# ttanida/rgrg

Hardware: AMD Instinct MI355X
Metric: images/sec full 29-region report gen, 512x512 CXR, greedy max_len=128 (higher is better)
Workload: dtype bf16; 1 GPU; full_model.generate() batch=32/GPU, 29 regions, greedy max_len=128, bf16 autocast: 16-bit detector, 16-bit decode GEMMs + K/V cache, hipGraph-captured decode step (BASELINE configs[2]); global_batch=32, parallelism=single GPU, weights=seeded random init (rgrg_amd.synth, profile bench), hipGraph_decode=True

## Files before the change

include/rgrg_hip.h:

```cpp
#ifndef RGRG_HIP_H_
#define RGRG_HIP_H_

#include <stdint.h>

#ifdef __cplusplus
extern "C" {
#endif

#define RGRG_OK 0
#define RGRG_EINVAL (-1)
#define RGRG_EHIP (-2)
#define RGRG_ESTATE (-3)

#define RGRG_ACT_NONE 0
#define RGRG_ACT_RELU 1
#define RGRG_ACT_GELU_NEW 2

const char* rgrg_last_error(void);
int rgrg_abi_version(void);
int rgrg_device_arch(int dev, char* buf, int buflen);

int rgrg_linear_f32(const float* A, const float* W, const float* scale, const float* shift, const float* R,
                    float* Y, int M, int N, int K, int ldy, int act, int splitk, float* ws, void* stream);
int rgrg_conv2d_nhwc_f32(const float* X, const float* W, const float* scale, const float* shift, const float* R,
// ... 68 lines not shown
                                  int* launches_per_step);
int rgrg_dropout_mask_f32(uint64_t seed, uint32_t stream_id, float p, int64_t n, int row_len, float* out, void* stream);
int rgrg_decoder_forward_cached(rgrg_decoder* d, const float* feats, const int64_t* input_ids, const int64_t* position_ids,
                                const float* attention_mask,
                                int S, int T, int past_len, float* logits_out, void* stream);
int rgrg_decoder_cache_plane(rgrg_decoder* d, int layer, int kv, void** ptr, int* max_seqs, int* slots, int* is_bf16);
int rgrg_decoder_take_id_error(rgrg_decoder* d, int* pending);
int rgrg_decoder_refresh_trainable(rgrg_decoder* d, void* stream);
int rgrg_transpose_pad_f32(const float* src, float* dst, int rows, int cols, int rows_padded, void* stream);
int rgrg_colsum_f32(const float* src, float* out, int rows, int cols, void* stream);
int rgrg_relu_backward_f32(float* d, const float* h, int64_t n, void* stream);
int rgrg_bce_with_logits_masked_backward_f32(const float* logits, const uint8_t* mask, const uint8_t* target, float pos_weight,
                                             int n, float scale, float* dlogits, int ld, void* stream);
int rgrg_adamw_step_f32(float* param, const float* grad, float* exp_avg, float* exp_avg_sq, int64_t n, float lr, float beta1,
                        float beta2, float eps, float weight_decay, int step, float grad_scale, void* stream);
int rgrg_adamw_multi_step_f32(const void* items, int n_items, float lr, float beta1, float beta2, float eps,
                              float weight_decay, int step, float grad_scale, void* stream);
int rgrg_f32_to_bf16(const float* src, uint16_t* dst, int64_t n, int fp16, void* stream);
int rgrg_bf16_to_f32(const uint16_t* src, float* dst, int64_t n, int fp16, void* stream);
int rgrg_conv2d_nhwc_bf16(const uint16_t* X16, const uint16_t* Wb, const float* shift, const uint16_t* R16, float* Y,
                          uint16_t* Y16, int B, int H, int Wd, int Cin, int Cout, int KH, int KW, int stride, int pad,
                          int act, int fp16, void* stream);
int rgrg_linear_bf16w_f32(const float* A, const uint16_t* Wb, const float* shift, const float* R, float* Y, int M,
                          int N, int K, int ldy, int act, int fp16, void* stream);
int rgrg_linear_bf16_f32(const uint16_t* A16, const uint16_t* Wb, const float* shift, const float* R, float* Y,
                         uint16_t* Y16, int M, int N, int K, int ldy, int act, int fp16, void* stream);
int rgrg_debug_linear_bf16_tile(const uint16_t* A16, const uint16_t* Wb, const float* shift, const float* R, float* Y,
                                int M, int N, int K, int ldy, int act, int tile, int lda, int ldw, int fp16, void* stream);
int rgrg_debug_linear_bf16_train(const uint16_t* A16, const uint16_t* Wb, const float* shift, const float* R, float* Y,
                                 uint16_t* Y16, uint16_t* Ypre16, const uint16_t* G16, int M, int N, int K, int ldy, int act,
                                 int tile, int fp16, void* stream);
int rgrg_debug_linear_bf16_argmax(const uint16_t* A16, const uint16_t* Wb, const float* shift, int M, int N, int K,
                                  float* cand_val, int* cand_idx, int fp16, void* stream);
int rgrg_debug_ln_fold16(const float* w, const float* gain, const float* beta, const float* bias, uint16_t* wb, float* colsum,
                         float* shift, int N, int K, int fp16, void* stream);
int rgrg_debug_linear_bf16_ln(const uint16_t* A16, const uint16_t* Wb, const float* shift, const float* R, float* Y,
                              uint16_t* Yb16, float* stats_out, const float* ln_stats, const float* ln_colsum, int M, int N,
                              int K, int ldy, int act, int fp16, void* stream);
int rgrg_debug_linear_bf16_ln_kp(const uint16_t* A16, const uint16_t* Wb, const float* shift, const float* R, float* Y,
                                 uint16_t* Y16, uint16_t* Yb16, float* stats_out, const float* ln_stats, const float* ln_colsum,
                                 int M, int N, int K, int ldy, int act, int fp16, int kp, void* stream);
int rgrg_box_match_f32(const float* gt, const int* gt_count, int G, const float* boxes, int64_t box_image_stride,
                       const int* box_count, int B, int N, float high, float low, int allow_low_quality, int* matched,
                       int* ws_best_per_gt, void* stream);
int rgrg_balanced_sample(const int* matched, const int64_t* gt_labels, int G, const int* box_count, const float* keys,
                         uint64_t seed, int stage, int B, int n, int batch, int max_pos, uint32_t* ws_keys, uint8_t* mask,
                         int* list, int* count, void* stream);
int rgrg_rpn_loss_sampled_f32(const float* rpn_out, int ld, int anchors_per_cell, const int* matched, const float* gt, int G,
                              const float* anchors, const uint8_t* mask, const int* list, const int* count, int B, int A,
                              int batch, float* out2, void* stream);
int rgrg_roi_add_gt_f32(const float* props, const int* counts, int P, const float* gt, const int* gt_count, int G, int B,
                        float* boxes, int* box_count, void* stream);
int rgrg_roi_gather_samples_f32(const float* boxes, const int* matched, const float* gt, const int64_t* gt_labels,
                                const int* gt_count, int G, const int* list, const int* count, int B, int N, int K, float wx,
                                float wy, float ww, float wh, float* props_s, int* offsets, int64_t* labels_flat,
                                float* reg_targets, void* stream);
int rgrg_fastrcnn_loss_f32(const float* pred, int ld, int num_classes, const int64_t* labels, const float* reg_targets, int N,
                           float* out2, void* stream);

int rgrg_decoder_copy_last_logits(rgrg_decoder* d, float* dst, int S, void* stream);
int rgrg_decoder_time_step_parts(rgrg_decoder* d, int S, int nkeys, int iters, int one_range, float* ms_gemm, float* ms_attn,
                                 double* gemm_flops, double* gemm_weight_bytes, double* kv_bytes, int* gemm_launches);
int rgrg_decoder_trace_step(rgrg_decoder* d, int S, int nkeys, int iters, float* recs, int max_recs, int* n_out);
int rgrg_decoder_attention_only(rgrg_decoder* d, int S, int nkeys, int iters, void* stream);
int rgrg_decoder_row_limit(rgrg_decoder* d);
int rgrg_debug_chain(int n, int mode, int blocks, float* us_per_kernel);
// ... 6 lines not shown
```

rgrg_amd/_hip.py:

```python
from __future__ import annotations

import ctypes as C
import os
from typing import Optional

from . import build as _build

c_float_p = C.c_void_p
_i, _f, _p = C.c_int, C.c_float, C.c_void_p

ACT_NONE, ACT_RELU, ACT_GELU_NEW = 0, 1, 2
ABI_VERSION = 21


class RgrgHipError(RuntimeError):
    pass


class DecoderLayerWeights(C.Structure):
    _fields_ = [(n, _p) for n in ("ln1_g", "ln1_b", "ln2_g", "ln2_b", "c_attn_w", "c_attn_b", "attn_proj_w",
                                  "attn_proj_b", "c_fc_w", "c_fc_b", "mlp_proj_w", "mlp_proj_b")]


class DecoderWeights(C.Structure):
# ... 16 lines not shown
    "rgrg_top1_per_class_f32": (_i, [_p, _i, _p, _p, _p, _p, _p, _p, _p, _i, _i, _i, _f, _f, _p]),
    "rgrg_select_regions_f32": (_i, [_p, _p, _f, _p, _p, _p, _i, _p]),
    "rgrg_bce_with_logits_masked_f32": (_i, [_p, _p, _p, C.c_float, _i, _p, _p]),
    "rgrg_preprocess_u8_f32": (_i, [_p, _i, _i, _i, _i, _i, C.c_float, C.c_float, _p, _p]),
    "rgrg_gather_rows_f32": (_i, [_p, _p, _p, _i, _i, _p]),
    "rgrg_decoder_create": (_i, [C.POINTER(DecoderWeights), _i, _i, C.POINTER(_p)]),
    "rgrg_decoder_create_with_cache": (_i, [C.POINTER(DecoderWeights), _i, _i, _p, C.c_size_t, C.POINTER(_p)]),
    "rgrg_decoder_kv_cache_bytes": (C.c_size_t, [_i, _i, _i]),
    "rgrg_decoder_destroy": (None, [_p]),
    "rgrg_decoder_generate": (_i, [_p, _p, _i, _i, _p, _i, C.POINTER(_i), _i, _p]),
    "rgrg_decoder_beam_search": (_i, [_p, _p, _i, _i, _i, _i, _f, _i, _p, _i, C.POINTER(_i), _p]),
    "rgrg_decoder_set_precision": (_i, [_p, _i]),
    "rgrg_decoder_lm_forward": (_i, [_p, _p, _p, _p, _i, _i, _p, _p, _p]),
    "rgrg_decoder_lm_loss_grad": (_i, [_p, _p, _p, _p, _i, _i, C.c_float, C.c_float, C.c_uint64, _p, _p, _p, _p, _p, _p, _p, _p]),
    "rgrg_dropout_mask_f32": (_i, [C.c_uint64, C.c_uint32, C.c_float, C.c_int64, _i, _p, _p]),
    "rgrg_decoder_refresh_trainable": (_i, [_p, _p]),
    "rgrg_decoder_take_id_error": (_i, [_p, C.POINTER(_i)]),
    "rgrg_decoder_forward_cached": (_i, [_p, _p, _p, _p, _p, _i, _i, _i, _p, _p]),
    "rgrg_decoder_cache_plane": (_i, [_p, _i, _i, C.POINTER(C.c_void_p), C.POINTER(_i), C.POINTER(_i), C.POINTER(_i)]),
    "rgrg_transpose_pad_f32": (_i, [_p, _p, _i, _i, _i, _p]),
    "rgrg_colsum_f32": (_i, [_p, _p, _i, _i, _p]),
    "rgrg_relu_backward_f32": (_i, [_p, _p, C.c_int64, _p]),
    "rgrg_bce_with_logits_masked_backward_f32": (_i, [_p, _p, _p, C.c_float, _i, C.c_float, _p, _i, _p]),
    "rgrg_adamw_step_f32": (_i, [_p, _p, _p, _p, C.c_int64, C.c_float, C.c_float, C.c_float, C.c_float, C.c_float, _i, C.c_float, _p]),
    "rgrg_adamw_multi_step_f32": (_i, [_p, _i, C.c_float, C.c_float, C.c_float, C.c_float, C.c_float, _i, C.c_float, _p]),
    "rgrg_f32_to_bf16": (_i, [_p, _p, C.c_int64, _i, _p]),
    "rgrg_bf16_to_f32": (_i, [_p, _p, C.c_int64, _i, _p]),
    "rgrg_conv2d_nhwc_bf16": (_i, [_p, _p, _p, _p, _p, _p, _i, _i, _i, _i, _i, _i, _i, _i, _i, _i, _i, _p]),
    "rgrg_linear_bf16w_f32": (_i, [_p, _p, _p, _p, _p, _i, _i, _i, _i, _i, _i, _p]),
    "rgrg_linear_bf16_f32": (_i, [_p, _p, _p, _p, _p, _p, _i, _i, _i, _i, _i, _i, _p]),
    "rgrg_debug_linear_bf16_tile": (_i, [_p, _p, _p, _p, _p, _i, _i, _i, _i, _i, _i, _i, _i, _i, _p]),
    "rgrg_debug_linear_bf16_train": (_i, [_p, _p, _p, _p, _p, _p, _p, _p, _i, _i, _i, _i, _i, _i, _i, _p]),
    "rgrg_debug_linear_bf16_argmax": (_i, [_p, _p, _p, _i, _i, _i, _p, _p, _i, _p]),
    "rgrg_debug_ln_fold16": (_i, [_p, _p, _p, _p, _p, _p, _p, _i, _i, _i, _p]),
    "rgrg_debug_linear_bf16_ln": (_i, [_p, _p, _p, _p, _p, _p, _p, _p, _p, _i, _i, _i, _i, _i, _i, _p]),
    "rgrg_debug_linear_bf16_ln_kp": (_i, [_p, _p, _p, _p, _p, _p, _p, _p, _p, _p, _i, _i, _i, _i, _i, _i, _i, _p]),
    "rgrg_decoder_copy_last_logits": (_i, [_p, _p, _i, _p]),
    "rgrg_box_match_f32": (_i, [_p, _p, _i, _p, C.c_int64, _p, _i, _i, _f, _f, _i, _p, _p, _p]),
    "rgrg_balanced_sample": (_i, [_p, _p, _i, _p, _p, C.c_uint64, _i, _i, _i, _i, _i, _p, _p, _p, _p, _p]),
    "rgrg_rpn_loss_sampled_f32": (_i, [_p, _i, _i, _p, _p, _i, _p, _p, _p, _p, _i, _i, _i, _p, _p]),
    "rgrg_roi_add_gt_f32": (_i, [_p, _p, _i, _p, _p, _i, _i, _p, _p, _p]),
    "rgrg_roi_gather_samples_f32": (_i, [_p, _p, _p, _p, _p, _i, _p, _p, _i, _i, _i, _f, _f, _f, _f, _p, _p, _p, _p, _p]),
    "rgrg_fastrcnn_loss_f32": (_i, [_p, _i, _i, _p, _p, _i, _p, _p]),
    "rgrg_decoder_trace_step": (_i, [_p, _i, _i, _i, _p, _i, C.POINTER(_i)]),
    "rgrg_decoder_attention_only": (_i, [_p, _i, _i, _i, _p]),
    "rgrg_decoder_row_limit": (_i, [_p]),
    "rgrg_decoder_set_lm_positions": (_i, [_p, _p, C.c_int64]),
    "rgrg_decoder_time_step_parts": (_i, [_p, _i, _i, _i, _i, C.POINTER(_f), C.POINTER(_f), C.POINTER(C.c_double),
                                          C.POINTER(C.c_double), C.POINTER(C.c_double), C.POINTER(_i)]),
    "rgrg_decoder_time_train_gemms": (_i, [_p, _i, _i, _i, C.POINTER(_f), C.POINTER(C.c_double), C.POINTER(_i)]),
    "rgrg_debug_chain": (_i, [_i, _i, _i, C.POINTER(_f)]),
}

_lib: Optional[C.CDLL] = None


def library_path() -> str:
    return _build.LIB_PATH


def load() -> C.CDLL:
    global _lib
    if _lib is not None:
        return _lib
    path = library_path()
    if _build.is_stale():
# ... 41 lines not shown
```

rgrg_amd/csrc/decoder.hip:

```cpp
#include <math.h>
#include <stdlib.h>

#include <algorithm>
#include <type_traits>
#include <cmath>
#include <vector>

#include "common.h"

namespace rgrg {

struct GemmParams;
int launch_gemm_dense(const float* A, const float* W, const float* shift, const float* R, float* Y, int M, int N, int K,
                      int ldy, int act, float* ws, size_t ws_floats, hipStream_t st);
int init_gemm_attrs();
int init_gemm_bf16_attrs();
struct GemmLnFold {
    void* Yb16 = nullptr;
    float* stats_out = nullptr;
    const float* ln_stats = nullptr;
    const float* ln_colsum = nullptr;
    void* Ypre16 = nullptr;
    const void* G16 = nullptr;
    int ksplit = 0;
    float* sk_ws = nullptr;
    unsigned* sk_cnt = nullptr;
    float* cand_val = nullptr;
    int* cand_idx = nullptr;
    int kp = 0;
};
bool gemm_bf16_cand_epilogue_ok(int M, int N, int K);
int launch_gemm_bf16w_ex(const float* A, const void* A16, const void* Wb, const float* shift, const float* R, float* Y, void* Y16,
                         int M, int N, int K, int ldy, int act, hipStream_t st, int f16, const GemmLnFold* ln = nullptr);
int launch_gemm_bf16w(const float* A, const void* Wb, const float* shift, const float* R, float* Y, int M, int N, int K,
                      int ldy, int act, hipStream_t st, int f16);
int convert_f32_to_bf16(const float* src, void* dst, size_t n, hipStream_t st, int f16);

constexpr int MAX_CHAINS = 4;
constexpr int PAD_ROWS = 32;
constexpr int SKINNY_MAX_ROWS = 128;
static int skinny_max_rows() {
    static int v = -1;
    if (v < 0) { const char* e = getenv("RGRG_SKINNY_MAX_ROWS"); v = e ? atoi(e) : SKINNY_MAX_ROWS;
        if (v > SKINNY_MAX_ROWS) v = SKINNY_MAX_ROWS; if (v < 32) v = 32; }
    return v;
}
constexpr int BOS_ID = 50256, EOS_ID = 50256, PAD_ID = 50256;
constexpr float LN_EPS = 1e-5f;

__global__ __launch_bounds__(256) void pack_weights_kernel(const float* __restrict__ W, float* __restrict__ P, int N,
                                                           int K, int NT) {
    const size_t total = (size_t)NT * (K / 8) * 64;
    for (size_t o = (size_t)blockIdx.x * blockDim.x + threadIdx.x; o < total; o += (size_t)gridDim.x * blockDim.x) {
        const int l = (int)(o & 63);
        const size_t t = o >> 6;
        const int kc = (int)(t % (K / 8));
        const int nt = (int)(t / (K / 8));
        const int n = nt * 32 + (l & 31);
        f32x4 v = {0.f, 0.f, 0.f, 0.f};
        if (n < N) v = *reinterpret_cast<const f32x4*>(W + (size_t)n * K + kc * 8 + (l >> 5) * 4);
        reinterpret_cast<f32x4*>(P)[o] = v;
    }
}

struct SkinnyArgs {
    const float* X;
    const float* P;
    const float* bias;
    const float* R;
    float* Y;
    float* part;
// ... 415 lines not shown
            L += pl[k] * wgt;
            o += pacc[k][threadIdx.x] * wgt;
        }
        out[frag_out ? frag_off(s, hd * 64 + threadIdx.x, D) : (size_t)s * D + hd * 64 + threadIdx.x] = o / L;
    }
}

typedef unsigned short u16;
typedef unsigned int u32x4 __attribute__((ext_vector_type(4)));
template <bool F16>
__device__ __forceinline__ float pair_lo(unsigned u) {
    if constexpr (F16) return f16_bits_to_f32(u & 0xffffu);
    else return __uint_as_float(u << 16);
}
template <bool F16>
__device__ __forceinline__ float pair_hi(unsigned u) {
    if constexpr (F16) return f16_bits_to_f32(u >> 16);
    else return __uint_as_float(u & 0xffff0000u);
}

struct Kv16Row {
    f32x4 q0, q1, k0, k1, v0, v1;
};
template <bool F16>
__device__ __forceinline__ u32x4 kv16_pack_round(const f32x4& lo, const f32x4& hi) {
    u32x4 o;
    o[0] = to16<F16>(lo[0]) | (to16<F16>(lo[1]) << 16);
    o[1] = to16<F16>(lo[2]) | (to16<F16>(lo[3]) << 16);
    o[2] = to16<F16>(hi[0]) | (to16<F16>(hi[1]) << 16);
    o[3] = to16<F16>(hi[2]) | (to16<F16>(hi[3]) << 16);
    return o;
}

template <int NI, bool HAS_SRC, bool FIRST, bool F16>
__device__ __forceinline__ void kv16_wave_chunk(const __amdgpu_buffer_rsrc_t kc, const __amdgpu_buffer_rsrc_t vc, const int* __restrict__ srow,
                                                int s, int hd, int H, int T, int base, int nkeys, int slot, int g, int d8,
                                                Kv16Row& r, float (&q)[8], u32x4& kn16, u32x4& vn16, float& m, float& l, float (&acc)[8]) {
    int rowi[NI];
#pragma unroll
    for (int i = 0; i < NI; ++i) rowi[i] = HAS_SRC ? srow[min(base + i * 8 + g, nkeys - 1)] : s;
    u32x4 kk[NI], vv[NI];
#pragma unroll
    for (int i = 0; i < NI; ++i) {
        const int jc = min(base + i * 8 + g, nkeys - 1);
        const unsigned off = ((unsigned)((rowi[i] * H + hd) * T + jc) * 64u + (unsigned)d8 * 8u) * 2u;
        kk[i] = __builtin_bit_cast(u32x4, __builtin_amdgcn_raw_buffer_load_b128(kc, (int)off, 0, 2));
        vv[i] = __builtin_bit_cast(u32x4, __builtin_amdgcn_raw_buffer_load_b128(vc, (int)off, 0, 2));
    }
    __builtin_amdgcn_sched_barrier(0);
    if constexpr (FIRST) {
#pragma unroll
        for (int e = 0; e < 4; ++e)
            asm volatile("" : "+v"(r.q0[e]), "+v"(r.q1[e]), "+v"(r.k0[e]), "+v"(r.k1[e]), "+v"(r.v0[e]), "+v"(r.v1[e]));
#pragma unroll
        for (int e = 0; e < 4; ++e) { q[e] = r.q0[e]; q[4 + e] = r.q1[e]; }
        kn16 = kv16_pack_round<F16>(r.k0, r.k1);
        vn16 = kv16_pack_round<F16>(r.v0, r.v1);
    }
    float sc[NI];
    float cmax = -INFINITY;
#pragma unroll
    for (int i = 0; i < NI; ++i) {
        const int j = base + i * 8 + g;
        if (j == slot) { kk[i] = kn16; vv[i] = vn16; }
        float dot = 0.f;
#pragma unroll
        for (int e = 0; e < 4; ++e)
            dot += q[2 * e] * pair_lo<F16>(kk[i][e]) + q[2 * e + 1] * pair_hi<F16>(kk[i][e]);
        dot += dpp_get<0xB1, 0xf>(dot);
        dot += dpp_get<0x4E, 0xf>(dot);
        dot += dpp_get<0x141, 0xf>(dot);
        sc[i] = j < nkeys ? dot / 8.0f : -INFINITY;
        cmax = fmaxf(cmax, sc[i]);
    }
    const float m_new = fmaxf(m, cmax);
    const float scale = (m == -INFINITY) ? 0.f : expf(m - m_new);
    const bool any = m_new != -INFINITY;
    l *= scale;
#pragma unroll
    for (int e = 0; e < 8; ++e) acc[e] *= scale;
#pragma unroll
    for (int i = 0; i < NI; ++i) {
        const int j = base + i * 8 + g;
        const float pj = (j < nkeys && any) ? expf(sc[i] - m_new) : 0.f;
        l += pj;
#pragma unroll
        for (int e = 0; e < 4; ++e) {
            const unsigned u = j < nkeys ? vv[i][e] : 0u;
            acc[2 * e] += pj * pair_lo<F16>(u);
            acc[2 * e + 1] += pj * pair_hi<F16>(u);
        }
    }
    m = m_new;
}

template <bool HAS_SRC, bool F16>
__global__ __launch_bounds__(256) void attn_decode_kv16_wave_kernel(const float* __restrict__ qkv, int ld_qkv,
                                                                    u16* __restrict__ kc, u16* __restrict__ vc,
                                                                    const int* __restrict__ step, float* __restrict__ out,
                                                                    int S, int H, int T, const int* __restrict__ src,
                                                                    u16* __restrict__ out16) {
    const int lane = threadIdx.x & 63;
    const int t = *step, nkeys = t + 2, slot = t + 1;
    const int g = lane >> 3, d8 = lane & 7;
    const int D = H * 64;
    const __amdgpu_buffer_rsrc_t rk = dx_rsrc(kc), rv = dx_rsrc(vc);
    for (int item = blockIdx.x * 4 + (threadIdx.x >> 6); item < S * H; item += gridDim.x * 4) {
    const int s = item / H, hd = item - s * H;
    const float* row = qkv + (size_t)s * ld_qkv;
    const int* srow = HAS_SRC ? src + (size_t)s * T : nullptr;
    Kv16Row r;
    r.q0 = *reinterpret_cast<const f32x4*>(row + hd * 64 + d8 * 8);
    r.q1 = *reinterpret_cast<const f32x4*>(row + hd * 64 + d8 * 8 + 4);
    r.k0 = *reinterpret_cast<const f32x4*>(row + D + hd * 64 + d8 * 8);
    r.k1 = *reinterpret_cast<const f32x4*>(row + D + hd * 64 + d8 * 8 + 4);
    r.v0 = *reinterpret_cast<const f32x4*>(row + 2 * D + hd * 64 + d8 * 8);
    r.v1 = *reinterpret_cast<const f32x4*>(row + 2 * D + hd * 64 + d8 * 8 + 4);
    float m = -INFINITY, l = 0.f, acc[8], q[8];
    u32x4 kn16, vn16;
#pragma unroll
    for (int e = 0; e < 8; ++e) acc[e] = 0.f;
#define KV16_CHUNK(NI_, FIRST_, BASE_) \
    kv16_wave_chunk<NI_, HAS_SRC, FIRST_, F16>(rk, rv, srow, s, hd, H, T, BASE_, nkeys, slot, g, d8, r, q, kn16, vn16, m, l, acc)
#define KV16_TAIL(FIRST_, BASE_, REM_)                                                                   \
    switch (((REM_) + 7) >> 3) {                                                                         \
        case 1: KV16_CHUNK(1, FIRST_, BASE_); break;                                                     \
        case 2: KV16_CHUNK(2, FIRST_, BASE_); break;                                                     \
        case 3: KV16_CHUNK(3, FIRST_, BASE_); break;                                                     \
        case 4: KV16_CHUNK(4, FIRST_, BASE_); break;                                                     \
        case 5: KV16_CHUNK(5, FIRST_, BASE_); break;                                                     \
        case 6: KV16_CHUNK(6, FIRST_, BASE_); break;                                                     \
        case 7: KV16_CHUNK(7, FIRST_, BASE_); break;                                                     \
        case 8: KV16_CHUNK(8, FIRST_, BASE_); break;                                                     \
        default: KV16_CHUNK(9, FIRST_, BASE_); break;                                                    \
    }
    if (nkeys > 72) {
        KV16_CHUNK(9, true, 0);
        int base = 72;
        for (; nkeys - base > 72; base += 72) KV16_CHUNK(9, false, base);
        KV16_TAIL(false, base, nkeys - base)
    } else {
        KV16_TAIL(true, 0, nkeys)
    }
#undef KV16_TAIL
#undef KV16_CHUNK
    if (g == 0) {
        const size_t o = (((size_t)s * H + hd) * T + slot) * 64 + d8 * 8;
        *reinterpret_cast<u32x4*>(kc + o) = kn16;
        *reinterpret_cast<u32x4*>(vc + o) = vn16;
    }
    float M = fmaxf(m, dpp_get<0x128, 0xf>(m));
    M = fmaxf(M, __shfl_xor(M, 16, 64));
    M = fmaxf(M, __shfl_xor(M, 32, 64));
    const float wgt = (m == -INFINITY) ? 0.f : expf(m - M);
    l *= wgt;
    l += dpp_get<0x128, 0xf>(l);
    l += __shfl_xor(l, 16, 64);
    l += __shfl_xor(l, 32, 64);
#pragma unroll
    for (int e = 0; e < 8; ++e) {
        float o = acc[e] * wgt;
        o += dpp_get<0x128, 0xf>(o);
        o += __shfl_xor(o, 16, 64);
        o += __shfl_xor(o, 32, 64);
        acc[e] = o / l;
    }
    if (g == 0) {
        const size_t o = (size_t)s * D + hd * 64 + d8 * 8;
        if (out16) {
            u32x4 pk;
#pragma unroll
            for (int i = 0; i < 4; ++i) pk[i] = to16<F16>(acc[2 * i]) | (to16<F16>(acc[2 * i + 1]) << 16);
            *reinterpret_cast<u32x4*>(out16 + o) = pk;
        } else {
            *reinterpret_cast<f32x4*>(out + o) = f32x4{acc[0], acc[1], acc[2], acc[3]};
            *reinterpret_cast<f32x4*>(out + o + 4) = f32x4{acc[4], acc[5], acc[6], acc[7]};
        }
    }
    }
}

template <typename KV>
__global__ __launch_bounds__(256) void kv_slot0_kernel(const float* __restrict__ ukv, int ld, KV* __restrict__ kv_all,
                                                       size_t layer_stride, size_t kv_stride, int S, int H, int T,
                                                       int L, int row_mul, int f16) {
    const int D = H * 64;
    const size_t total = (size_t)L * 2 * S * D;
    for (size_t i = (size_t)blockIdx.x * blockDim.x + threadIdx.x; i < total; i += (size_t)gridDim.x * blockDim.x) {
        const int d = (int)(i % D);
        size_t r = i / D;
        const int s = (int)(r % S);
        r /= S;
        const int kv = (int)(r & 1), l = (int)(r >> 1);
        const int hd = d >> 6, e = d & 63;
        const float val = ukv[(size_t)s * ld + ((size_t)l * 2 + kv) * D + d];
        const size_t o = (size_t)l * layer_stride + (size_t)kv * kv_stride + (((size_t)s * row_mul * H + hd) * T) * 64 + e;
        if constexpr (sizeof(KV) == 2) kv_all[o] = (KV)to16_rt(val, f16);
        else kv_all[o] = val;
    }
}

constexpr int ARGMAX_U = 13;
__global__ __launch_bounds__(256) void argmax_update_kernel(const float* __restrict__ cand_val, const int* __restrict__ cand_idx,
                                                            int NT, long long* __restrict__ ids, int ld_ids,
                                                            int* __restrict__ finished, int* __restrict__ step,
                                                            int* __restrict__ done_len, int* __restrict__ sync, int S) {
    __shared__ float bv[4];
    __shared__ int bi[4];
    const int row = blockIdx.x, tid = threadIdx.x, lane = tid & 63, wave = tid >> 6;
    const int t = *step;
    const float* cv = cand_val + (size_t)row * NT;
// ... 923 lines not shown
            GemmLnFold f = *ln;
            f.ln_colsum = l.cs16;
            f.kp = (d->kp_gemms == 1 || d->kp_gemms == 3) ? 1 : 0;
            return launch_gemm_bf16w_ex(nullptr, X16, l.wb_ln, l.c2_16, R, Y16 ? nullptr : Y, Y16, M, l.N, l.K, ldy, act, d->stream, d->f16(), &f);
        }
        if (ln && ln->Yb16 && d->sk_ws && M <= d->rows) {
            int ks = l.K >= 2048 ? d->sk_mlp : d->sk_attn;
            if (ks < 0) ks = (d->step_rows > 0 && d->step_rows <= 256) ? (l.K >= 2048 ? 4 : 2) : 1;
            if (ks > 1) {
                GemmLnFold f = *ln;
                const size_t r0 = d->xn16 ? (size_t)(reinterpret_cast<const unsigned short*>(ln->Yb16) - d->xn16) / (size_t)d->D : 0;
                const size_t tile0 = (r0 / 64) * (size_t)(l.N / 64);
                f.ksplit = ks; f.sk_ws = d->sk_ws + tile0 * 4 * 4096; f.sk_cnt = d->sk_cnt + tile0;
                return launch_gemm_bf16w_ex(nullptr, X16, l.wb, l.b, R, Y16 ? nullptr : Y, Y16, M, l.N, l.K, ldy, act, d->stream, d->f16(), &f);
            }
        }
        if (ln && ln->Yb16 && X16 && (d->kp_gemms == 1 || d->kp_gemms == 2)) {
            GemmLnFold f = *ln;
            f.kp = 1;
            return launch_gemm_bf16w_ex(nullptr, X16, l.wb, l.b, R, Y16 ? nullptr : Y, Y16, M, l.N, l.K, ldy, act, d->stream, d->f16(), &f);
        }
        return launch_gemm_bf16w_ex(X16 ? nullptr : X, X16, l.wb, l.b, R, Y16 ? nullptr : Y, Y16, M, l.N, l.K, ldy, act, d->stream, d->f16(), ln);
    }
    if (count) d->gemm_bytes_per_step += (size_t)l.N * l.K * sizeof(float);
    return launch_gemm_dense(X, l.w, l.b, R, Y, M, l.N, l.K, ldy, act, d->gemm_ws, d->gemm_ws_floats, d->stream);
}


static bool lm_head_cand_path(const rgrg_decoder* d, int S) {
    return S > decode_row_limit(d) && kv_is_bf16(d, S) && d->xn16 && d->lm_head.wb && d->lm_head.K % 256 == 0 &&
           gemm_bf16_cand_epilogue_ok(S, d->lm_head.N, d->lm_head.K);
}

static int launch_attention(rgrg_decoder* d, int l, int S, const int* src, unsigned short* att16, int frag_out = 0, int r0 = 0) {
    hipStream_t st = d->stream;
    const int D = d->D;
    float* kc = d->kv + (size_t)l * d->kv_layer_stride;
    float* vc = kc + d->kv_kv_stride;
    if (kv_is_bf16(d, S)) {
        u16* kc16 = reinterpret_cast<u16*>(d->kv) + (size_t)l * d->kv_layer_stride;
        if ((d->H & 3) != 0 || (size_t)d->kv_kv_stride * sizeof(u16) >= ((size_t)1 << 31)) {
            set_error("decoder: the bf16 K/V cache plane of one layer (%zu bytes) exceeds the 2 GiB the attention kernel addresses: "
                      "lower the batch or max_length", (size_t)d->kv_kv_stride * sizeof(u16));
            return RGRG_EINVAL;
        }
        static const int cap = [] { const char* e = getenv("RGRG_ATTN_WGS_PER_CU"); return e ? atoi(e) : 0; }();
        const int wgs = S * d->H / 4;
        const dim3 wgrid(cap > 0 ? std::min(wgs, cap * 256) : wgs), wblk(256);
        u16* kc16r = kc16 + (size_t)r0 * d->H * d->T * 64;
#define KV16_LAUNCH(SRC_, F16_) hipLaunchKernelGGL((attn_decode_kv16_wave_kernel<SRC_, F16_>), wgrid, wblk, 0, st, d->qkv + (size_t)r0 * 3 * D, 3 * D, kc16r, \
                                                  kc16r + d->kv_kv_stride, d->step, d->att + (size_t)r0 * D, S, d->H, d->T, src, att16)
        if (src) { if (d->f16()) KV16_LAUNCH(true, true); else KV16_LAUNCH(true, false); }
        else { if (d->f16()) KV16_LAUNCH(false, true); else KV16_LAUNCH(false, false); }
#undef KV16_LAUNCH
    } else {
        const dim3 grid(S * d->H), blk(256);
#define ATT_LAUNCH(SRC_, NI_) hipLaunchKernelGGL((attn_decode_kernel<SRC_, NI_>), grid, blk, 0, st, d->qkv, 3 * D, kc, vc, d->step, d->att, S, d->H, d->T, src, frag_out)
        if (d->key_mask_cur && !src) {
#define ATT_LAUNCH_MASK(NI_) hipLaunchKernelGGL((attn_decode_kernel<false, NI_, true>), grid, blk, 0, st, d->qkv, 3 * D, kc, vc, d->step, d->att, S, d->H, d->T, \
                                                  src, frag_out, d->key_mask_cur)
            if (S * d->H <= 4096) ATT_LAUNCH_MASK(9); else ATT_LAUNCH_MASK(2);
#undef ATT_LAUNCH_MASK
        } else if (S * d->H <= 4096) { if (src) ATT_LAUNCH(true, 9); else ATT_LAUNCH(false, 9); }
        else { if (src) ATT_LAUNCH(true, 2); else ATT_LAUNCH(false, 2); }
#undef ATT_LAUNCH
    }
    RGRG_LAUNCH_CHECK();
    return RGRG_OK;
}

static int direct_linear(rgrg_decoder* d, const Lin& l, DirectArgs a, int mode, int M, bool count, bool cand = false) {
    if (!l.direct) { set_error("direct_linear: layer was not packed for the fused plan"); return RGRG_EINVAL; }
    if (l.lnf && mode == DX_PLAIN && !a.Xf) { set_error("direct_linear: missing operand"); return RGRG_EINVAL; }
    a.P = l.packed; a.bias = l.lnf ? l.c2 : l.b; a.c1 = l.c1;
    a.M = M; a.K = l.K; a.N = l.N; a.NT = l.NT; a.KS = l.KS;
    if (l.KS > 1) a.part_out = d->part;
    if (cand) { a.cand_val = d->cand_val; a.cand_idx = d->cand_idx; }
    const int mt = (M + PAD_ROWS - 1) / PAD_ROWS;
    const int w16 = (d->bf16_gemms && d->w16_fused && mt > 1 && l.packed16 && l.packed16_f16 == d->f16() && (!l.lnf || l.c1_16)) ? (d->f16() ? 2 : 1) : 0;
    if (w16) { a.P = reinterpret_cast<const float*>(l.packed16); if (l.lnf) a.c1 = l.c1_16; }
    const dim3 grid(l.NT, l.KS), blk(64 * SK_WAVES);
    hipStream_t st = d->stream;
    if (l.lnf && mode == DX_COMBINE4 && l.NT > 512 && mt == 1 && l.K == DK_SLICE) {
        hipLaunchKernelGGL((rgrg_lm_head_wave_f32<DX_COMBINE4>), dim3(256), blk, LMH_LDS, st, a);
    } else if (!l.lnf && mode == DX_PLAIN && l.KS == 1 && mt == 1 && l.NT <= 64 && M > 16 && !cand) {
        hipLaunchKernelGGL(rgrg_skinny_direct_half_f32, dim3(l.NT, 2), blk, 0, st, a);
    } else {
// ... 1324 lines not shown
    return RGRG_OK;
}

extern "C" int rgrg_decoder_take_id_error(rgrg_decoder* d, int* pending) {
    RGRG_CHECK_ARG(d && pending);
    RGRG_HIP(hipStreamSynchronize(d->stream));
    *pending = (d->h_id_error && *d->h_id_error) ? 1 : 0;
    if (*pending) {
        *d->h_id_error = 0;
        RGRG_HIP(hipMemsetAsync(d->id_error, 0, 2 * sizeof(int), d->stream));
    }
    return RGRG_OK;
}

extern "C" int rgrg_decoder_refresh_trainable(rgrg_decoder* d, void* stream) {
    RGRG_CHECK_ARG(d);
    hipStream_t caller = as_stream(stream), st = d->stream;
    RGRG_HIP(hipEventRecord(d->ev_in, caller));
    RGRG_HIP(hipStreamWaitEvent(st, d->ev_in, 0));
    Lin* ls[] = {&d->fst0, &d->fst2, &d->ukv};
    for (Lin* l : ls) {
        if (l->packed) {
            hipLaunchKernelGGL(pack_weights_kernel, dim3(2048), dim3(256), 0, st, l->w, l->packed, l->N, l->K, l->NT);
            RGRG_LAUNCH_CHECK();
        }
        if (l->wT) {
            int rc = launch_transpose_pad(l->w, l->wT, l->N, l->K, pad256(l->N), st);
            if (rc) return rc;
        }
    }
    RGRG_HIP(hipEventRecord(d->ev_in, st));
    RGRG_HIP(hipStreamWaitEvent(caller, d->ev_in, 0));
    return RGRG_OK;
}

extern "C" int rgrg_debug_ln_fold16(const float* w, const float* gain, const float* beta, const float* bias, uint16_t* wb,
                                    float* colsum, float* shift, int N, int K, int fp16, void* stream) {
    RGRG_CHECK_ARG(w && gain && beta && wb && colsum && shift && N > 0 && K > 0);
    hipLaunchKernelGGL(ln_fold16_kernel, dim3((N + 3) / 4), dim3(256), 0, as_stream(stream), w, gain, beta, bias, wb, colsum, shift, N, K,
                       fp16 ? 1 : 0);
    RGRG_LAUNCH_CHECK();
    return RGRG_OK;
}

static int set_precision_impl(rgrg_decoder* d, int mode);
extern "C" int rgrg_decoder_set_precision(rgrg_decoder* d, int mode) {
    RGRG_CHECK_ARG(d && mode >= 0 && mode <= 2);
    if (mode == d->bf16_gemms) return RGRG_OK;
    const int prev = d->bf16_gemms;
    const int rc = set_precision_impl(d, mode);
    if (rc) {
        auto stale = [](Lin& l) { l.wb_f16 = -1; l.wb_ln_f16 = -1; l.wTb_f16 = -1; };
        stale(d->lm_head); stale(d->ukv); stale(d->fst2);
        for (auto& w : d->layers) { stale(w.c_attn); stale(w.attn_proj); stale(w.c_fc); stale(w.mlp_proj); }
        d->bf16_gemms = 0;
        (void)prev;
        for (auto& g : d->graphs) (void)hipGraphExecDestroy(g.exec);
        d->graphs.clear();
    }
    return rc;
}
static int set_precision_impl(rgrg_decoder* d, int mode) {
    d->logits_valid = false;
    const int prev = d->bf16_gemms;
    d->bf16_gemms = mode;
    if (mode) {
// ... 257 lines not shown
```

Baseline: 86.26 images/sec.

## Software-pipeline kv16 decode attention across items with persistent occupancy-sized grid

Restructures the bf16 K/V-cache decode attention kernel so each wave double-buffers its work items. It issues the Q/K/V row loads and first-chunk cache loads for the next (sequence, head) item before doing the math for the current one. The grid is now capped at a configurable number of waves per SIMD times the CU count, so waves loop over items persistently instead of one item per wave. This is meant to hide global/buffer load latency, at the cost of more live registers (two buffers of up to 9 K/V vectors) and possible lower occupancy or imbalance. It also adds a debug entry point for the kernel.

After: 78.28 images/sec (median of 2 runs). 0.907x the previous value.

```diff
diff --git a/include/rgrg_hip.h b/include/rgrg_hip.h
--- a/include/rgrg_hip.h
+++ b/include/rgrg_hip.h
@@ -124,6 +124,8 @@
                                  int tile, int fp16, void* stream);
 int rgrg_debug_linear_bf16_argmax(const uint16_t* A16, const uint16_t* Wb, const float* shift, int M, int N, int K,
                                   float* cand_val, int* cand_idx, int fp16, void* stream);
+int rgrg_debug_attn_decode_kv16(const float* qkv, int ld_qkv, uint16_t* k_cache, uint16_t* v_cache, const int* step, float* out,
+                                uint16_t* out16, int S, int H, int T, const int* src, int fp16, void* stream);
 int rgrg_debug_ln_fold16(const float* w, const float* gain, const float* beta, const float* bias, uint16_t* wb, float* colsum,
                          float* shift, int N, int K, int fp16, void* stream);
 int rgrg_debug_linear_bf16_ln(const uint16_t* A16, const uint16_t* Wb, const float* shift, const float* R, float* Y,
diff --git a/rgrg_amd/_hip.py b/rgrg_amd/_hip.py
--- a/rgrg_amd/_hip.py
+++ b/rgrg_amd/_hip.py
@@ -72,6 +72,7 @@
     "rgrg_debug_linear_bf16_tile": (_i, [_p, _p, _p, _p, _p, _i, _i, _i, _i, _i, _i, _i, _i, _i, _p]),
     "rgrg_debug_linear_bf16_train": (_i, [_p, _p, _p, _p, _p, _p, _p, _p, _i, _i, _i, _i, _i, _i, _i, _p]),
     "rgrg_debug_linear_bf16_argmax": (_i, [_p, _p, _p, _i, _i, _i, _p, _p, _i, _p]),
+    "rgrg_debug_attn_decode_kv16": (_i, [_p, _i, _p, _p, _p, _p, _p, _i, _i, _i, _p, _i, _p]),
     "rgrg_debug_ln_fold16": (_i, [_p, _p, _p, _p, _p, _p, _p, _i, _i, _i, _p]),
     "rgrg_debug_linear_bf16_ln": (_i, [_p, _p, _p, _p, _p, _p, _p, _p, _p, _i, _i, _i, _i, _i, _i, _p]),
     "rgrg_debug_linear_bf16_ln_kp": (_i, [_p, _p, _p, _p, _p, _p, _p, _p, _p, _p, _i, _i, _i, _i, _i, _i, _i, _p]),
diff --git a/rgrg_amd/csrc/decoder.hip b/rgrg_amd/csrc/decoder.hip
--- a/rgrg_amd/csrc/decoder.hip
+++ b/rgrg_amd/csrc/decoder.hip
@@ -37,6 +37,7 @@
 int convert_f32_to_bf16(const float* src, void* dst, size_t n, hipStream_t st, int f16);
 
 constexpr int MAX_CHAINS = 4;
+constexpr int ATTN_WAVES_PER_SIMD = 2;
 constexpr int PAD_ROWS = 32;
 constexpr int SKINNY_MAX_ROWS = 128;
 static int skinny_max_rows() {
@@ -518,14 +519,14 @@
     return o;
 }
 
-template <int NI, bool HAS_SRC, bool FIRST, bool F16>
-__device__ __forceinline__ void kv16_wave_chunk(const __amdgpu_buffer_rsrc_t kc, const __amdgpu_buffer_rsrc_t vc, const int* __restrict__ srow,
-                                                int s, int hd, int H, int T, int base, int nkeys, int slot, int g, int d8,
-                                                Kv16Row& r, float (&q)[8], u32x4& kn16, u32x4& vn16, float& m, float& l, float (&acc)[8]) {
-    int rowi[NI];
+template <int NI, bool HAS_SRC>
+__device__ __forceinline__ void kv16_rows(const int* __restrict__ srow, int s, int base, int nkeys, int g, int (&rowi)[NI]) {
 #pragma unroll
     for (int i = 0; i < NI; ++i) rowi[i] = HAS_SRC ? srow[min(base + i * 8 + g, nkeys - 1)] : s;
-    u32x4 kk[NI], vv[NI];
+}
+template <int NI>
+__device__ __forceinline__ void kv16_load(const __amdgpu_buffer_rsrc_t kc, const __amdgpu_buffer_rsrc_t vc, const int (&rowi)[NI],
+                                          int hd, int H, int T, int base, int nkeys, int g, int d8, u32x4 (&kk)[NI], u32x4 (&vv)[NI]) {
 #pragma unroll
     for (int i = 0; i < NI; ++i) {
         const int jc = min(base + i * 8 + g, nkeys - 1);
@@ -533,11 +534,13 @@
         kk[i] = __builtin_bit_cast(u32x4, __builtin_amdgcn_raw_buffer_load_b128(kc, (int)off, 0, 2));
         vv[i] = __builtin_bit_cast(u32x4, __builtin_amdgcn_raw_buffer_load_b128(vc, (int)off, 0, 2));
     }
-    __builtin_amdgcn_sched_barrier(0);
+}
+
+template <int NI, bool FIRST, bool F16>
+__device__ __forceinline__ void kv16_chunk_math(u32x4 (&kk)[NI], u32x4 (&vv)[NI], int base, int nkeys, int slot, int g,
+                                                const Kv16Row& r, float (&q)[8], u32x4& kn16, u32x4& vn16, float& m, float& l,
+                                                float (&acc)[8]) {
     if constexpr (FIRST) {
-#pragma unroll
-        for (int e = 0; e < 4; ++e)
-            asm volatile("" : "+v"(r.q0[e]), "+v"(r.q1[e]), "+v"(r.k0[e]), "+v"(r.k1[e]), "+v"(r.v0[e]), "+v"(r.v1[e]));
 #pragma unroll
         for (int e = 0; e < 4; ++e) { q[e] = r.q0[e]; q[4 + e] = r.q1[e]; }
         kn16 = kv16_pack_round<F16>(r.k0, r.k1);
@@ -580,60 +583,87 @@
     m = m_new;
 }
 
-template <bool HAS_SRC, bool F16>
-__global__ __launch_bounds__(256) void attn_decode_kv16_wave_kernel(const float* __restrict__ qkv, int ld_qkv,
-                                                                    u16* __restrict__ kc, u16* __restrict__ vc,
-                                                                    const int* __restrict__ step, float* __restrict__ out,
-                                                                    int S, int H, int T, const int* __restrict__ src,
-                                                                    u16* __restrict__ out16) {
-    const int lane = threadIdx.x & 63;
-    const int t = *step, nkeys = t + 2, slot = t + 1;
-    const int g = lane >> 3, d8 = lane & 7;
-    const int D = H * 64;
-    const __amdgpu_buffer_rsrc_t rk = dx_rsrc(kc), rv = dx_rsrc(vc);
-    for (int item = blockIdx.x * 4 + (threadIdx.x >> 6); item < S * H; item += gridDim.x * 4) {
-    const int s = item / H, hd = item - s * H;
-    const float* row = qkv + (size_t)s * ld_qkv;
-    const int* srow = HAS_SRC ? src + (size_t)s * T : nullptr;
+struct Kv16Args {
+    const float* qkv;
+    const int* src;
+    float* out;
+    u16* kc;
+    u16* vc;
+    u16* out16;
+    __amdgpu_buffer_rsrc_t rk, rv;
+    int ld_qkv, H, T, D, n, nkeys, slot, g, d8;
+};
+template <int NI, bool HAS_SRC>
+struct Kv16Loc {
+    int s, hd;
+    int rowi[NI];
+};
+template <int NI>
+struct Kv16Buf {
+    int s, hd;
     Kv16Row r;
-    r.q0 = *reinterpret_cast<const f32x4*>(row + hd * 64 + d8 * 8);
-    r.q1 = *reinterpret_cast<const f32x4*>(row + hd * 64 + d8 * 8 + 4);
-    r.k0 = *reinterpret_cast<const f32x4*>(row + D + hd * 64 + d8 * 8);
-    r.k1 = *reinterpret_cast<const f32x4*>(row + D + hd * 64 + d8 * 8 + 4);
-    r.v0 = *reinterpret_cast<const f32x4*>(row + 2 * D + hd * 64 + d8 * 8);
-    r.v1 = *reinterpret_cast<const f32x4*>(row + 2 * D + hd * 64 + d8 * 8 + 4);
+    u32x4 kk[NI], vv[NI];
+};
+
+template <int NI, bool HAS_SRC>
+__device__ __forceinline__ void kv16_locate(const Kv16Args& a, Kv16Loc<NI, HAS_SRC>& L, int item) {
+    L.s = item / a.H;
+    L.hd = item - L.s * a.H;
+    kv16_rows<NI, HAS_SRC>(HAS_SRC ? a.src + (size_t)L.s * a.T : nullptr, L.s, 0, a.nkeys, a.g, L.rowi);
+}
+template <int NI, bool HAS_SRC>
+__device__ __forceinline__ void kv16_issue(const Kv16Args& a, Kv16Buf<NI>& b, const Kv16Loc<NI, HAS_SRC>& L) {
+    b.s = L.s;
+    b.hd = L.hd;
+    const float* row = a.qkv + (size_t)b.s * a.ld_qkv + b.hd * 64 + a.d8 * 8;
+    b.r.q0 = *reinterpret_cast<const f32x4*>(row);
+    b.r.q1 = *reinterpret_cast<const f32x4*>(row + 4);
+    b.r.k0 = *reinterpret_cast<const f32x4*>(row + a.D);
+    b.r.k1 = *reinterpret_cast<const f32x4*>(row + a.D + 4);
+    b.r.v0 = *reinterpret_cast<const f32x4*>(row + 2 * a.D);
+    b.r.v1 = *reinterpret_cast<const f32x4*>(row + 2 * a.D + 4);
+    kv16_load<NI>(a.rk, a.rv, L.rowi, b.hd, a.H, a.T, 0, a.nkeys, a.g, a.d8, b.kk, b.vv);
+}
+
+template <int NI, bool HAS_SRC, bool F16>
+__device__ __forceinline__ void kv16_chunk(const Kv16Args& a, int s, int hd, int base, const Kv16Row& r, float (&q)[8],
+                                           u32x4& kn16, u32x4& vn16, float& m, float& l, float (&acc)[8]) {
+    int rowi[NI];
+    kv16_rows<NI, HAS_SRC>(HAS_SRC ? a.src + (size_t)s * a.T : nullptr, s, base, a.nkeys, a.g, rowi);
+    u32x4 kk[NI], vv[NI];
+    kv16_load<NI>(a.rk, a.rv, rowi, hd, a.H, a.T, base, a.nkeys, a.g, a.d8, kk, vv);
+    kv16_chunk_math<NI, false, F16>(kk, vv, base, a.nkeys, a.slot, a.g, r, q, kn16, vn16, m, l, acc);
+}
+
+template <int NI, bool MULTI, bool HAS_SRC, bool F16>
+__device__ __forceinline__ void kv16_finish(const Kv16Args& a, Kv16Buf<NI>& b) {
+    const int s = b.s, hd = b.hd, g = a.g, d8 = a.d8, nkeys = a.nkeys, slot = a.slot;
     float m = -INFINITY, l = 0.f, acc[8], q[8];
     u32x4 kn16, vn16;
 #pragma unroll
     for (int e = 0; e < 8; ++e) acc[e] = 0.f;
-#define KV16_CHUNK(NI_, FIRST_, BASE_) \
-    kv16_wave_chunk<NI_, HAS_SRC, FIRST_, F16>(rk, rv, srow, s, hd, H, T, BASE_, nkeys, slot, g, d8, r, q, kn16, vn16, m, l, acc)
-#define KV16_TAIL(FIRST_, BASE_, REM_)                                                                   \
-    switch (((REM_) + 7) >> 3) {                                                                         \
-        case 1: KV16_CHUNK(1, FIRST_, BASE_); break;                                                     \
-        case 2: KV16_CHUNK(2, FIRST_, BASE_); break;                                                     \
-        case 3: KV16_CHUNK(3, FIRST_, BASE_); break;                                                     \
-        case 4: KV16_CHUNK(4, FIRST_, BASE_); break;                                                     \
-        case 5: KV16_CHUNK(5, FIRST_, BASE_); break;                                                     \
-        case 6: KV16_CHUNK(6, FIRST_, BASE_); break;                                                     \
-        case 7: KV16_CHUNK(7, FIRST_, BASE_); break;                                                     \
-        case 8: KV16_CHUNK(8, FIRST_, BASE_); break;                                                     \
-        default: KV16_CHUNK(9, FIRST_, BASE_); break;                                                    \
-    }
-    if (nkeys > 72) {
-        KV16_CHUNK(9, true, 0);
+    kv16_chunk_math<NI, true, F16>(b.kk, b.vv, 0, nkeys, slot, g, b.r, q, kn16, vn16, m, l, acc);
+    if constexpr (MULTI) {
         int base = 72;
-        for (; nkeys - base > 72; base += 72) KV16_CHUNK(9, false, base);
-        KV16_TAIL(false, base, nkeys - base)
-    } else {
-        KV16_TAIL(true, 0, nkeys)
-    }
+        for (; nkeys - base > 72; base += 72) kv16_chunk<9, HAS_SRC, F16>(a, s, hd, base, b.r, q, kn16, vn16, m, l, acc);
+#define KV16_TAIL(NI_) kv16_chunk<NI_, HAS_SRC, F16>(a, s, hd, base, b.r, q, kn16, vn16, m, l, acc)
+        switch ((nkeys - base + 7) >> 3) {
+            case 1: KV16_TAIL(1); break;
+            case 2: KV16_TAIL(2); break;
+            case 3: KV16_TAIL(3); break;
+            case 4: KV16_TAIL(4); break;
+            case 5: KV16_TAIL(5); break;
+            case 6: KV16_TAIL(6); break;
+            case 7: KV16_TAIL(7); break;
+            case 8: KV16_TAIL(8); break;
+            default: KV16_TAIL(9); break;
+        }
 #undef KV16_TAIL
-#undef KV16_CHUNK
+    }
     if (g == 0) {
-        const size_t o = (((size_t)s * H + hd) * T + slot) * 64 + d8 * 8;
-        *reinterpret_cast<u32x4*>(kc + o) = kn16;
-        *reinterpret_cast<u32x4*>(vc + o) = vn16;
+        const size_t o = (((size_t)s * a.H + hd) * a.T + slot) * 64 + d8 * 8;
+        *reinterpret_cast<u32x4*>(a.kc + o) = kn16;
+        *reinterpret_cast<u32x4*>(a.vc + o) = vn16;
     }
     float M = fmaxf(m, dpp_get<0x128, 0xf>(m));
     M = fmaxf(M, __shfl_xor(M, 16, 64));
@@ -652,17 +682,71 @@
         acc[e] = o / l;
     }
     if (g == 0) {
-        const size_t o = (size_t)s * D + hd * 64 + d8 * 8;
-        if (out16) {
+        const size_t o = (size_t)s * a.D + hd * 64 + d8 * 8;
+        if (a.out16) {
             u32x4 pk;
 #pragma unroll
             for (int i = 0; i < 4; ++i) pk[i] = to16<F16>(acc[2 * i]) | (to16<F16>(acc[2 * i + 1]) << 16);
-            *reinterpret_cast<u32x4*>(out16 + o) = pk;
+            *reinterpret_cast<u32x4*>(a.out16 + o) = pk;
         } else {
-            *reinterpret_cast<f32x4*>(out + o) = f32x4{acc[0], acc[1], acc[2], acc[3]};
-            *reinterpret_cast<f32x4*>(out + o + 4) = f32x4{acc[4], acc[5], acc[6], acc[7]};
-        }
-    }
+            *reinterpret_cast<f32x4*>(a.out + o) = f32x4{acc[0], acc[1], acc[2], acc[3]};
+            *reinterpret_cast<f32x4*>(a.out + o + 4) = f32x4{acc[4], acc[5], acc[6], acc[7]};
+        }
+    }
+}
+
+template <int NI, bool MULTI, bool HAS_SRC, bool F16>
+__device__ __forceinline__ void kv16_items(const Kv16Args& a, int it, int stride) {
+    const int count = (a.n - it + stride - 1) / stride;
+    Kv16Loc<NI, HAS_SRC> la, lb;
+    Kv16Buf<NI> ba, bb;
+    kv16_locate(a, la, it);
+    kv16_locate(a, lb, it + stride < a.n ? it + stride : it);
+    kv16_issue(a, ba, la);
+    for (int p = 0; p < count / 2; ++p) {
+        kv16_locate(a, la, it + 2 * stride < a.n ? it + 2 * stride : it);
+        kv16_issue(a, bb, lb);
+        __builtin_amdgcn_sched_barrier(0);
+        kv16_finish<NI, MULTI, HAS_SRC, F16>(a, ba);
+        it += stride;
+        kv16_locate(a, lb, it + 2 * stride < a.n ? it + 2 * stride : it);
+        kv16_issue(a, ba, la);
+        __builtin_amdgcn_sched_barrier(0);
+        kv16_finish<NI, MULTI, HAS_SRC, F16>(a, bb);
+        it += stride;
+    }
+    if (count & 1) kv16_finish<NI, MULTI, HAS_SRC, F16>(a, ba);
+}
+
+template <bool HAS_SRC, bool F16>
+__global__ __launch_bounds__(256) void attn_decode_kv16_wave_kernel(const float* __restrict__ qkv, int ld_qkv,
+                                                                    u16* __restrict__ kc, u16* __restrict__ vc,
+                                                                    const int* __restrict__ step, float* __restrict__ out,
+                                                                    int S, int H, int T, const int* __restrict__ src,
+                                                                    u16* __restrict__ out16) {
+    const int lane = threadIdx.x & 63;
+    const int t = *step;
+    Kv16Args a;
+    a.qkv = qkv; a.src = src; a.out = out; a.kc = kc; a.vc = vc; a.out16 = out16;
+    a.rk = dx_rsrc(kc); a.rv = dx_rsrc(vc);
+    a.ld_qkv = ld_qkv; a.H = H; a.T = T; a.D = H * 64; a.n = S * H;
+    a.nkeys = t + 2; a.slot = t + 1; a.g = lane >> 3; a.d8 = lane & 7;
+    const int it = blockIdx.x * 4 + __builtin_amdgcn_readfirstlane(threadIdx.x >> 6), stride = gridDim.x * 4;
+    if (it >= a.n) return;
+    if (a.nkeys > 72) {
+        kv16_items<9, true, HAS_SRC, F16>(a, it, stride);
+        return;
+    }
+    switch ((a.nkeys + 7) >> 3) {
+        case 1: kv16_items<1, false, HAS_SRC, F16>(a, it, stride); break;
+        case 2: kv16_items<2, false, HAS_SRC, F16>(a, it, stride); break;
+        case 3: kv16_items<3, false, HAS_SRC, F16>(a, it, stride); break;
+        case 4: kv16_items<4, false, HAS_SRC, F16>(a, it, stride); break;
+        case 5: kv16_items<5, false, HAS_SRC, F16>(a, it, stride); break;
+        case 6: kv16_items<6, false, HAS_SRC, F16>(a, it, stride); break;
+        case 7: kv16_items<7, false, HAS_SRC, F16>(a, it, stride); break;
+        case 8: kv16_items<8, false, HAS_SRC, F16>(a, it, stride); break;
+        default: kv16_items<9, false, HAS_SRC, F16>(a, it, stride); break;
     }
 }
 
@@ -1652,6 +1736,22 @@
            gemm_bf16_cand_epilogue_ok(S, d->lm_head.N, d->lm_head.K);
 }
 
+static int launch_attn_kv16(const float* qkv, int ld_qkv, u16* kc, u16* vc, const int* step, float* out, u16* out16, int S, int H,
+                            int T, const int* src, bool f16, hipStream_t st) {
+    int dev = 0, cus = 0;
+    RGRG_HIP(hipGetDevice(&dev));
+    RGRG_HIP(hipDeviceGetAttribute(&cus, hipDeviceAttributeMultiprocessorCount, dev));
+    static const int wps = [] { const char* e = getenv("RGRG_ATTN_WAVES_PER_SIMD"); return e && atoi(e) > 0 ? atoi(e) : ATTN_WAVES_PER_SIMD; }();
+    const dim3 grid(std::min(S * H / 4, wps * std::max(cus, 1))), blk(256);
+#define KV16_LAUNCH(SRC_, F16_) \
+    hipLaunchKernelGGL((attn_decode_kv16_wave_kernel<SRC_, F16_>), grid, blk, 0, st, qkv, ld_qkv, kc, vc, step, out, S, H, T, src, out16)
+    if (src) { if (f16) KV16_LAUNCH(true, true); else KV16_LAUNCH(true, false); }
+    else { if (f16) KV16_LAUNCH(false, true); else KV16_LAUNCH(false, false); }
+#undef KV16_LAUNCH
+    RGRG_LAUNCH_CHECK();
+    return RGRG_OK;
+}
+
 static int launch_attention(rgrg_decoder* d, int l, int S, const int* src, unsigned short* att16, int frag_out = 0, int r0 = 0) {
     hipStream_t st = d->stream;
     const int D = d->D;
@@ -1664,15 +1764,9 @@
                       "lower the batch or max_length", (size_t)d->kv_kv_stride * sizeof(u16));
             return RGRG_EINVAL;
         }
-        static const int cap = [] { const char* e = getenv("RGRG_ATTN_WGS_PER_CU"); return e ? atoi(e) : 0; }();
-        const int wgs = S * d->H / 4;
-        const dim3 wgrid(cap > 0 ? std::min(wgs, cap * 256) : wgs), wblk(256);
         u16* kc16r = kc16 + (size_t)r0 * d->H * d->T * 64;
-#define KV16_LAUNCH(SRC_, F16_) hipLaunchKernelGGL((attn_decode_kv16_wave_kernel<SRC_, F16_>), wgrid, wblk, 0, st, d->qkv + (size_t)r0 * 3 * D, 3 * D, kc16r, \
-                                                  kc16r + d->kv_kv_stride, d->step, d->att + (size_t)r0 * D, S, d->H, d->T, src, att16)
-        if (src) { if (d->f16()) KV16_LAUNCH(true, true); else KV16_LAUNCH(true, false); }
-        else { if (d->f16()) KV16_LAUNCH(false, true); else KV16_LAUNCH(false, false); }
-#undef KV16_LAUNCH
+        return launch_attn_kv16(d->qkv + (size_t)r0 * 3 * D, 3 * D, kc16r, kc16r + d->kv_kv_stride, d->step, d->att + (size_t)r0 * D,
+                                att16, S, d->H, d->T, src, d->f16(), st);
     } else {
         const dim3 grid(S * d->H), blk(256);
 #define ATT_LAUNCH(SRC_, NI_) hipLaunchKernelGGL((attn_decode_kernel<SRC_, NI_>), grid, blk, 0, st, d->qkv, 3 * D, kc, vc, d->step, d->att, S, d->H, d->T, src, frag_out)
@@ -3063,6 +3157,13 @@
     RGRG_HIP(hipEventRecord(d->ev_in, st));
     RGRG_HIP(hipStreamWaitEvent(caller, d->ev_in, 0));
     return RGRG_OK;
+}
+
+extern "C" int rgrg_debug_attn_decode_kv16(const float* qkv, int ld_qkv, uint16_t* k_cache, uint16_t* v_cache, const int* step,
+                                           float* out, uint16_t* out16, int S, int H, int T, const int* src, int fp16, void* stream) {
+    RGRG_CHECK_ARG(qkv && k_cache && v_cache && step && (out || out16) && S > 0 && H > 0 && H % 4 == 0 && T >= 2 &&
+                   ld_qkv >= 3 * H * 64 && (size_t)S * H * T * 64 * sizeof(uint16_t) < ((size_t)1 << 31));
+    return launch_attn_kv16(qkv, ld_qkv, k_cache, v_cache, step, out, out16, S, H, T, src, fp16 != 0, as_stream(stream));
 }
 
 extern "C" int rgrg_debug_ln_fold16(const float* w, const float* gain, const float* beta, const float* bias, uint16_t* wb,
```
